# imdea-software/legosnark

Hardware: AMD Instinct MI355X
Metric: alt_bn128 G1 MSM point-scalar pairs/s at n=2^20 (higher is better)
Workload: dtype u32 limbs (254-bit Montgomery integers)

## Files before the change

legosnark_amd/csrc/msm.hip:

```cpp
#include <hip/hip_runtime.h>
#include <stdint.h>
#include <stdio.h>
#include <stdlib.h>
#include <string.h>
#include <algorithm>
#include <type_traits>
#include <vector>

#include "curves.h"
#include "fp29x2l.h"
#include "fs29.h"
#include "glv.h"
#include "msm.h"
#include "msm_plan.h"

namespace lsa {


template <class F, int K>
__global__ __launch_bounds__(256) void k_normalize(const Jac<F> *__restrict__ in, Aff<F> *__restrict__ out, size_t n) {
    size_t t = (size_t)blockIdx.x * blockDim.x + threadIdx.x;
    size_t base = t * K;
    if (base >= n) return;
    F prod[K];
// ... 198 lines not shown
__device__ __forceinline__ uint32_t block_exclusive_scan_256(uint32_t v, uint32_t *lds, uint32_t *total) {
    const unsigned lane = threadIdx.x & 63, wv = threadIdx.x >> 6;
    uint32_t incl = v;
#pragma unroll
    for (int d = 1; d < 64; d <<= 1) {
        uint32_t t = __shfl_up(incl, d, 64);
        if ((int)lane >= d) incl += t;
    }
    if (lane == 63) lds[wv] = incl;
    __syncthreads();
    uint32_t base = 0, tot = 0;
#pragma unroll
    for (unsigned w = 0; w < 4; w++) { uint32_t x = lds[w]; if (w < wv) base += x; tot += x; }
    __syncthreads();
    *total = tot;
    return base + incl - v;
}

__global__ __launch_bounds__(256) void k_scan_sums(const uint32_t *__restrict__ hist, uint32_t count, uint32_t *__restrict__ block_sums) {
    __shared__ uint32_t lds[4];
    const uint32_t base = blockIdx.x * SCAN_PER_BLOCK + threadIdx.x * 8;
    uint32_t s = 0;
#pragma unroll
    for (int j = 0; j < 8; j++) if (base + j < count) s += hist[base + j];
    uint32_t tot;
    (void)block_exclusive_scan_256(s, lds, &tot);
    if (threadIdx.x == 0) block_sums[blockIdx.x] = tot;
}

__global__ __launch_bounds__(256) void k_scan_blocks(uint32_t *__restrict__ block_sums, uint32_t nblocks) {
    __shared__ uint32_t lds[4];
    uint32_t v[4], s = 0;
#pragma unroll
    for (int j = 0; j < 4; j++) { uint32_t idx = threadIdx.x * 4 + j; v[j] = idx < nblocks ? block_sums[idx] : 0; s += v[j]; }
    uint32_t tot;
    uint32_t run = block_exclusive_scan_256(s, lds, &tot);
#pragma unroll
    for (int j = 0; j < 4; j++) { uint32_t idx = threadIdx.x * 4 + j; if (idx < nblocks) block_sums[idx] = run; run += v[j]; }
}

__global__ __launch_bounds__(256) void k_scan_final(const uint32_t *__restrict__ hist, const uint32_t *__restrict__ block_sums,
                                                    uint32_t count, uint32_t *__restrict__ offs) {
    __shared__ uint32_t lds[4];
    const uint32_t base = blockIdx.x * SCAN_PER_BLOCK + threadIdx.x * 8;
    uint32_t v[8], s = 0;
#pragma unroll
    for (int j = 0; j < 8; j++) { v[j] = (base + j < count) ? hist[base + j] : 0; s += v[j]; }
    uint32_t tot;
    uint32_t run = block_sums[blockIdx.x] + block_exclusive_scan_256(s, lds, &tot);
#pragma unroll
    for (int j = 0; j < 8; j++) { if (base + j < count) offs[base + j] = run; run += v[j]; }
}

__global__ __launch_bounds__(1024) void k_scatter(const int32_t *__restrict__ digits, const uint16_t *__restrict__ rank,
                                                  const uint32_t *__restrict__ offs, const uint32_t *__restrict__ tile_base,
                                                  size_t n, size_t npoints, uint32_t B, uint32_t ntiles, uint32_t *__restrict__ entries,
                                                  uint32_t win_stride) {
    extern __shared__ __attribute__((aligned(16))) uint32_t base[];
    const uint32_t t = blockIdx.x, k = blockIdx.y;
    const uint32_t *of = offs + (size_t)k * B;
    const uint32_t *tb = tile_base + ((size_t)k * ntiles + t) * B;
    for (uint32_t x = threadIdx.x; x < B; x += 1024) base[x] = of[x] + tb[x];
    __syncthreads();
    const size_t lo = (size_t)t * SORT_TILE;
    const size_t hi = lo + SORT_TILE < n ? lo + SORT_TILE : n;
    const int32_t *dg = digits + (size_t)k * n;
    const uint16_t *rk = rank + (size_t)k * n;
    for (size_t i = lo + threadIdx.x; i < hi; i += 1024) {
        int32_t sd = dg[i];
        if (sd != 0) {
            uint32_t b = (uint32_t)(sd < 0 ? -sd : sd) - 1;
            uint32_t pt = i < npoints ? (uint32_t)i : ((uint32_t)(i - npoints) | 0x40000000u);
            pt += k * win_stride;
            entries[base[b] + rk[i]] = pt | (sd < 0 ? 0x80000000u : 0u);
        }
    }
}

__global__ __launch_bounds__(1024) void k_tile_scan_rows(const uint16_t *__restrict__ tile_hist, uint32_t Bc, uint32_t R, uint32_t pitch,
                                                         uint32_t *__restrict__ tile_base, uint32_t *__restrict__ hist,
                                                         uint32_t *__restrict__ zero1, uint32_t *__restrict__ zeron, uint32_t nzero) {
    __builtin_amdgcn_s_setprio(3);
    if (blockIdx.x == 0) {
        if (threadIdx.x == 0) *zero1 = 0;
        for (uint32_t x = threadIdx.x; x < nzero; x += 1024) zeron[x] = 0;
    }
    __shared__ uint32_t part[32][33];
    const unsigned lane = threadIdx.x & 63, wv = threadIdx.x >> 6;
    const unsigned bl = lane & 31, grp = 2 * wv + (lane >> 5);
    const uint32_t b = blockIdx.x * 32 + bl;
    const uint32_t per = (R + 31) / 32, r0 = grp * per, r1 = r0 + per < R ? r0 + per : R;
    constexpr uint32_t MAXPER = 16;
    uint32_t v[MAXPER];
    uint32_t sum = 0;
    const bool in_regs = per <= MAXPER;
    if (in_regs) {
#pragma unroll
        for (uint32_t j = 0; j < MAXPER; j++) {
            const uint32_t r = r0 + j;
            v[j] = (b < Bc && r < r1) ? tile_hist[(size_t)r * pitch + b] : 0u;
        }
#pragma unroll
        for (uint32_t j = 0; j < MAXPER; j++) sum += v[j];
    } else if (b < Bc) {
        for (uint32_t r = r0; r < r1; r++) sum += tile_hist[(size_t)r * pitch + b];
    }
    part[grp][bl] = sum;
    __syncthreads();
    uint32_t run = 0, tot = 0;
#pragma unroll
    for (unsigned g2 = 0; g2 < 32; g2++) { uint32_t x = part[g2][bl]; if (g2 < grp) run += x; tot += x; }
    if (b < Bc) {
        if (in_regs) {
#pragma unroll
            for (uint32_t j = 0; j < MAXPER; j++) {
                const uint32_t r = r0 + j;
                if (r < r1) { tile_base[(size_t)r * pitch + b] = run; run += v[j]; }
            }
        } else {
            for (uint32_t r = r0; r < r1; r++) {
                const size_t idx = (size_t)r * pitch + b;
                tile_base[idx] = run;
                run += tile_hist[idx];
            }
        }
        if (grp == 0) hist[b] = tot;
    }
}

__device__ __forceinline__ uint32_t segment_of(const SegList &segs, uint32_t i) {
    uint32_t seg = 0;
    for (uint32_t j = 1; j < segs.nseg; j++) if (i >= segs.off[j]) seg = j;
    return seg;
}

__device__ __forceinline__ uint32_t xcd_tile(uint32_t bid, uint32_t ntiles) {
    const uint32_t q = ntiles >> 3, r = ntiles & 7u, x = bid & 7u, j = bid >> 3;
    return x * q + (x < r ? x : r) + j;
}

__global__ __launch_bounds__(1024) void k_hist_wide(const Fr *__restrict__ scalars, size_t n, SegList segs, WidePlan pl, uint32_t B,
                                                    uint32_t Bc, CoarseMap cm, uint32_t pitch, uint32_t tile,
                                                    uint16_t *__restrict__ tile_hist) {
    __builtin_amdgcn_s_setprio(3);
    extern __shared__ __attribute__((aligned(16))) uint32_t cnt2[];
    for (uint32_t x = threadIdx.x; x < (Bc + 1) / 2; x += blockDim.x) cnt2[x] = 0;
    __syncthreads();
    const uint32_t t = xcd_tile(blockIdx.x, gridDim.x);
    const size_t lo = (size_t)t * tile;
    for (uint32_t il = threadIdx.x; il < tile; il += blockDim.x) {
        const size_t i = lo + il;
        if (i >= n) break;
        const uint32_t seg = segment_of(segs, (uint32_t)i);
        wide_digits(scalars[i], pl, seg * B, [&](unsigned, int32_t sd) {
            if (sd != 0) {
                const uint32_t b = cm.bin((uint32_t)(sd < 0 ? -sd : sd) - 1);
                atomicAdd(&cnt2[b >> 1], 1u << ((b & 1) * 16));
            }
        });
    }
    __syncthreads();
    uint16_t *th = tile_hist + (size_t)t * pitch;
    const uint16_t *c16 = reinterpret_cast<const uint16_t *>(cnt2);
    for (uint32_t x = threadIdx.x; x < Bc; x += blockDim.x) th[x] = c16[x];
}

template <int REC>
// ... 32 lines not shown
    const size_t lo = (size_t)t * tile;
    for (uint32_t il = threadIdx.x; il < tile; il += 1024) {
        const size_t i = lo + il;
        if (i >= n) break;
        const uint32_t seg = segment_of(segs, (uint32_t)i);
        const uint32_t local = (uint32_t)i - segs.off[seg];
        wide_digits(scalars[i], pl, seg * B, [&](unsigned k, int32_t sd) {
            if (sd != 0) {
                const uint32_t b = (uint32_t)(sd < 0 ? -sd : sd) - 1;
                const uint32_t ent = (local + k * win_stride) | (sd < 0 ? 0x80000000u : 0u);
                if (REC == 1) ((uint64_t *)out)[atomicAdd(&base[b >> 7], 1u)] = ((uint64_t)(b & 127u) << 32) | ent;
                else if (REC == 2) ((uint32_t *)out)[atomicAdd(&base[b >> 6], 1u)] = (ent & 0x81ffffffu) | ((b & 63u) << 25);
                else ((uint32_t *)out)[atomicAdd(&base[b], 1u)] = ent;
            }
        });
    }
}

__device__ __forceinline__ uint32_t lds_inc_rank(uint32_t *counters, uint32_t idx) {
    const uint32_t first = (uint32_t)__builtin_amdgcn_readfirstlane((int)idx);
    const uint64_t active = __ballot(1), same = __ballot(idx == first);
    if (same == active) {
        const uint32_t rank = __builtin_amdgcn_mbcnt_hi((uint32_t)(active >> 32), __builtin_amdgcn_mbcnt_lo((uint32_t)active, 0u));
        uint32_t base = 0;
        if (rank == 0) base = atomicAdd(&counters[first], (uint32_t)__popcll(active));
        return (uint32_t)__builtin_amdgcn_readfirstlane((int)base) + rank;
    }
    return atomicAdd(&counters[idx], 1u);
}
__global__ __launch_bounds__(1024) void k_partition(const Fr *__restrict__ scalars, size_t n, SegList segs, WidePlan pl, uint32_t B, uint32_t Bc,
                                                    CoarseMap cm, uint32_t pitch, const uint16_t *__restrict__ tile_hist,
                                                    const uint32_t *__restrict__ hist_c, uint32_t *__restrict__ offs_c,
                                                    const uint32_t *__restrict__ tile_base, uint32_t *__restrict__ recs) {
    __builtin_amdgcn_s_setprio(3);
    extern __shared__ __attribute__((aligned(16))) uint32_t stage[];
    __shared__ uint32_t lstart[PART_SEGS + 1], lcur[PART_SEGS], gdst[PART_SEGS], wtot[2][PART_SEGS / 64];
    const uint32_t t = xcd_tile(blockIdx.x, gridDim.x);
    const unsigned lane = threadIdx.x & 63, wv = threadIdx.x >> 6;
    {
        uint32_t gv = 0, lv = 0;
        if (threadIdx.x < Bc) { gv = hist_c[threadIdx.x]; lv = tile_hist[(size_t)t * pitch + threadIdx.x]; }
        uint32_t gi = gv, li = lv;
#pragma unroll
        for (int d = 1; d < 64; d <<= 1) {
            const uint32_t a = __shfl_up(gi, d, 64), b = __shfl_up(li, d, 64);
            if ((int)lane >= d) { gi += a; li += b; }
        }
        if (wv < PART_SEGS / 64 && lane == 63) { wtot[0][wv] = gi; wtot[1][wv] = li; }
        __syncthreads();
        if (threadIdx.x < Bc) {
            uint32_t gex = gi - gv, lex = li - lv;
            for (unsigned w = 0; w < wv; w++) { gex += wtot[0][w]; lex += wtot[1][w]; }
            lstart[threadIdx.x] = lex;
            lcur[threadIdx.x] = lex;
            gdst[threadIdx.x] = gex + tile_base[(size_t)t * pitch + threadIdx.x];
            if (blockIdx.x == 0) offs_c[threadIdx.x] = gex;
            if (threadIdx.x == Bc - 1) lstart[Bc] = lex + lv;
        }
    }
    __syncthreads();
    const size_t lo = (size_t)t * PART_TILE;
    const uint32_t fine_bits = cm.sh_hi;
    const uint32_t tlow = t & ((1u << (16 - fine_bits)) - 1);
    for (uint32_t j = 0; j < PART_TILE / 1024; j++) {
        const uint32_t il = threadIdx.x + j * 1024;
        const size_t i = lo + il;
        if (i >= n) break;
        const uint32_t seg = segment_of(segs, (uint32_t)i);
        wide_digits(scalars[i], pl, seg * B, [&](unsigned k, int32_t sd) {
            if (sd != 0) {
                const uint32_t b = (uint32_t)(sd < 0 ? -sd : sd) - 1;
                const uint32_t pos = atomicAdd(&lcur[cm.bin(b)], 1u);
                stage[pos] = (tlow << (16 + fine_bits)) | (cm.fine(b) << 16) | (k << 12) | (sd < 0 ? 0x800u : 0u) | il;
            }
        });
    }
    __syncthreads();
    for (uint32_t sg = threadIdx.x >> 5; sg < Bc; sg += 32) {
        const uint32_t a = lstart[sg], e = lstart[sg + 1], g = gdst[sg];
        for (uint32_t x = a + (lane & 31); x < e; x += 32) recs[g + (x - a)] = stage[x];
    }
}

__global__ __launch_bounds__(1024) void k_fine_sort_part(const uint32_t *__restrict__ recs, const uint32_t *__restrict__ offs_c,
                                                         const uint32_t *__restrict__ hist_c, const uint32_t *__restrict__ tile_base,
                                                         uint32_t pitch, uint32_t T, CoarseMap cm, SegList segs, uint32_t win_stride, uint32_t stage_cap,
                                                         uint32_t *__restrict__ entries, uint32_t *__restrict__ hist, uint32_t *__restrict__ offs) {
    __builtin_amdgcn_s_setprio(3);
    extern __shared__ __attribute__((aligned(16))) uint32_t sm[];
    __shared__ uint32_t wsum[16];
    const uint32_t sg = blockIdx.x, lo = offs_c[sg], ns = hist_c[sg];
    const uint32_t fine_bits = cm.sh_hi, FM = 1u << fine_bits, fmask = FM - 1, tbits = 16 - fine_bits;
    const uint32_t F = 1u << cm.bits(sg), bucket0 = cm.first(sg);
    uint32_t *cnt = sm, *cur = sm + FM, *col = sm + 2 * FM, *stage = col + T + 1;
    const unsigned lane = threadIdx.x & 63, wv = threadIdx.x >> 6;
    for (uint32_t x = threadIdx.x; x < F; x += 1024) cnt[x] = 0;
    for (uint32_t x = threadIdx.x; x < T; x += 1024) col[x] = tile_base[(size_t)x * pitch + sg];
    if (threadIdx.x == 0) col[T] = ns;
    auto scan_counters = [&]() {
        const uint32_t per = (F + 1023) >> 10, f0 = threadIdx.x * per;
        uint32_t sum = 0;
        for (uint32_t q = 0; q < per; q++) if (f0 + q < F) sum += cnt[f0 + q];
        uint32_t incl = sum;
#pragma unroll
        for (int d = 1; d < 64; d <<= 1) {
            const uint32_t u = __shfl_up(incl, d, 64);
            if ((int)lane >= d) incl += u;
        }
        if (lane == 63) wsum[wv] = incl;
        __syncthreads();
        uint32_t run = incl - sum;
        for (unsigned w = 0; w < wv; w++) run += wsum[w];
        for (uint32_t q = 0; q < per; q++) {
            if (f0 + q >= F) break;
            const uint32_t c = cnt[f0 + q];
            cur[f0 + q] = run;
            hist[(size_t)bucket0 + f0 + q] = c;
            offs[(size_t)bucket0 + f0 + q] = lo + run;
            run += c;
        }
    };
    auto entry_of = [&](uint32_t r, uint32_t p2) {
        uint32_t a = 0, e = (T + (1u << tbits) - 1) >> tbits;
        while (e - a > 1) {
            const uint32_t m = (a + e) >> 1;
            if (col[m << tbits] <= p2) a = m; else e = m;
        }
        const uint32_t i = ((a << tbits) | (r >> (16 + fine_bits))) * PART_TILE + (r & 0x7ffu);
        const uint32_t local = i - segs.off[segment_of(segs, i)];
        return (local + ((r >> 12) & 15u) * win_stride) | ((r & 0x800u) << 20);
    };
    if (ns <= stage_cap) {
        constexpr uint32_t NR = PART_STAGE / 1024;
        uint32_t r[NR];
#pragma unroll
        for (uint32_t u = 0; u < NR; u++) { const uint32_t p2 = threadIdx.x + u * 1024; r[u] = p2 < ns ? recs[lo + p2] : 0u; }
        __syncthreads();
        uint16_t rk[NR];
#pragma unroll
        for (uint32_t u = 0; u < NR; u++) {
            rk[u] = 0;
            if (threadIdx.x + u * 1024 < ns) rk[u] = (uint16_t)atomicAdd(&cnt[(r[u] >> 16) & fmask], 1u);
        }
        __syncthreads();
        scan_counters();
        __syncthreads();
#pragma unroll
        for (uint32_t u = 0; u < NR; u++) {
            const uint32_t p2 = threadIdx.x + u * 1024;
            if (p2 < ns) stage[cur[(r[u] >> 16) & fmask] + rk[u]] = entry_of(r[u], p2);
        }
        __syncthreads();
        for (uint32_t x = threadIdx.x; x < ns; x += 1024) entries[lo + x] = stage[x];
        return;
    }
    __syncthreads();
    constexpr uint32_t UNR = 8;
    for (uint32_t p0 = threadIdx.x; p0 < ns; p0 += 1024 * UNR) {
        uint32_t r[UNR];
#pragma unroll
        for (uint32_t u = 0; u < UNR; u++) { const uint32_t p2 = p0 + u * 1024; r[u] = p2 < ns ? recs[lo + p2] : 0u; }
#pragma unroll
        for (uint32_t u = 0; u < UNR; u++) if (p0 + u * 1024 < ns) (void)lds_inc_rank(cnt, (r[u] >> 16) & fmask);
    }
    __syncthreads();
    scan_counters();
    __syncthreads();
    for (uint32_t p0 = threadIdx.x; p0 < ns; p0 += 1024 * UNR) {
        uint32_t r[UNR];
#pragma unroll
        for (uint32_t u = 0; u < UNR; u++) { const uint32_t p2 = p0 + u * 1024; r[u] = p2 < ns ? recs[lo + p2] : 0u; }
#pragma unroll
        for (uint32_t u = 0; u < UNR; u++) {
            const uint32_t p2 = p0 + u * 1024;
            if (p2 >= ns) break;
            entries[lo + lds_inc_rank(cur, (r[u] >> 16) & fmask)] = entry_of(r[u], p2);
        }
    }
}

template <class Rec>
struct RecOps;
template <>
struct RecOps<uint64_t> {
    static constexpr uint32_t NF = 128;
    static __device__ __forceinline__ uint32_t fine(uint64_t r) { return (uint32_t)(r >> 32); }
    static __device__ __forceinline__ uint32_t entry(uint64_t r) { return (uint32_t)r; }
};
template <>
struct RecOps<uint32_t> {
    static constexpr uint32_t NF = 64;
    static __device__ __forceinline__ uint32_t fine(uint32_t r) { return (r >> 25) & 63u; }
    static __device__ __forceinline__ uint32_t entry(uint32_t r) { return r & 0x81ffffffu; }
};
template <class Rec>
__global__ __launch_bounds__(1024) void k_fine_sort(const Rec *__restrict__ recs, const uint32_t *__restrict__ offs_c,
                                                    const uint32_t *__restrict__ hist_c, uint32_t *__restrict__ entries,
                                                    uint32_t *__restrict__ hist, uint32_t *__restrict__ offs) {
    using O = RecOps<Rec>;
    constexpr uint32_t NF = O::NF;
    __shared__ uint32_t cnt[NF], cur[NF];
    const uint32_t bin = blockIdx.x, lo = offs_c[bin], n = hist_c[bin];
    if (threadIdx.x < NF) cnt[threadIdx.x] = 0;
    __syncthreads();
    for (uint32_t j = threadIdx.x; j < n; j += 1024) atomicAdd(&cnt[O::fine(recs[lo + j])], 1u);
    __syncthreads();
    if (threadIdx.x < 64) {
        constexpr uint32_t PER = NF / 64;
        uint32_t c[PER], tot = 0;
#pragma unroll
        for (uint32_t q = 0; q < PER; q++) { c[q] = cnt[PER * threadIdx.x + q]; tot += c[q]; }
        uint32_t incl = tot;
#pragma unroll
        for (int d = 1; d < 64; d <<= 1) {
            uint32_t t = __shfl_up(incl, d, 64);
            if ((int)threadIdx.x >= d) incl += t;
        }
        uint32_t ex = incl - tot;
#pragma unroll
        for (uint32_t q = 0; q < PER; q++) {
            cur[PER * threadIdx.x + q] = ex;
            hist[(size_t)bin * NF + PER * threadIdx.x + q] = c[q];
            offs[(size_t)bin * NF + PER * threadIdx.x + q] = lo + ex;
            ex += c[q];
        }
    }
    __syncthreads();
    for (uint32_t j = threadIdx.x; j < n; j += 1024) {
        const Rec r = recs[lo + j];
        const uint32_t pos = atomicAdd(&cur[O::fine(r)], 1u);
        entries[lo + pos] = O::entry(r);
    }
}

__device__ __forceinline__ uint32_t size_bin(uint32_t cnt, uint32_t bin_shift) { return ((cnt - 1) >> bin_shift) + 1; }
template <class C>
__global__ __launch_bounds__(256) void k_size_hist(const uint32_t *__restrict__ hist, uint32_t nb, uint32_t thr, uint32_t *__restrict__ bin_count,
                                                   uint32_t group_size, uint32_t bin_shift) {
    bin_count += (group_size ? (blockIdx.x * 2048u) / group_size : 0u) * SIZE_BINS;
    __shared__ uint32_t lcnt[SIZE_BINS];
    for (uint32_t t = threadIdx.x; t < SIZE_BINS; t += 256) lcnt[t] = 0;
    __syncthreads();
    const uint32_t base = blockIdx.x * 2048 + threadIdx.x;
#pragma unroll
    for (int j = 0; j < 8; j++) {
        uint32_t g = base + j * 256;
        if (g < nb) { uint32_t cnt = hist[g]; if (cnt > 0 && cnt <= thr) atomicAdd(&lcnt[size_bin(cnt, bin_shift)], 1u); }
    }
    __syncthreads();
    for (uint32_t t = threadIdx.x; t < SIZE_BINS; t += 256) if (lcnt[t]) atomicAdd(&bin_count[t], lcnt[t]);
}
__global__ __launch_bounds__(256) void k_size_scan(const uint32_t *__restrict__ bin_count, uint32_t *__restrict__ bin_start, uint32_t ngroups) {
    __shared__ uint32_t lds[4];
    uint32_t carry = 0;
    for (uint32_t gidx = 0; gidx < ngroups; gidx++) {
        const uint32_t *bc = bin_count + gidx * SIZE_BINS;
        uint32_t *bs = bin_start + gidx * SIZE_BINS;
        uint32_t v[4], s = 0;
#pragma unroll
        for (int j = 0; j < 4; j++) {
            int bin = (int)SIZE_BINS - 1 - (int)(threadIdx.x * 4 + j);
            v[j] = (bin >= 1) ? bc[bin] : 0;
            s += v[j];
        }
        uint32_t tot;
        uint32_t run = carry + block_exclusive_scan_256(s, lds, &tot);
#pragma unroll
        for (int j = 0; j < 4; j++) {
            int bin = (int)SIZE_BINS - 1 - (int)(threadIdx.x * 4 + j);
            if (bin >= 1) bs[bin] = run;
            run += v[j];
        }
        carry += tot;
    }
    if (threadIdx.x == 0) bin_start[0] = carry;
}
template <class C>
__global__ __launch_bounds__(256) void k_size_scatter(const uint32_t *__restrict__ hist, uint32_t nb, uint32_t thr, const uint32_t *__restrict__ bin_start,
                                                      uint32_t *__restrict__ bin_cursor, uint32_t *__restrict__ perm,
                                                      uint32_t *__restrict__ heavy_list, uint32_t *__restrict__ heavy_count,
                                                      typename C::Acc *__restrict__ buckets, uint32_t group_size, uint32_t bin_shift,
                                                      uint32_t split) {
    const uint32_t goff = (group_size ? (blockIdx.x * 2048u) / group_size : 0u) * SIZE_BINS;
    bin_start += goff;
    bin_cursor += goff;
    __shared__ uint32_t lcnt[SIZE_BINS];
    for (uint32_t t = threadIdx.x; t < SIZE_BINS; t += 256) lcnt[t] = 0;
    __syncthreads();
    const uint32_t base = blockIdx.x * 2048 + threadIdx.x;
    uint32_t cnt[8], rank[8];
#pragma unroll
    for (int j = 0; j < 8; j++) {
        uint32_t g = base + j * 256;
        cnt[j] = 0; rank[j] = 0;
        if (g < nb) {
            cnt[j] = hist[g];
            if (cnt[j] == 0) { for (uint32_t h = 0; h < split; h++) buckets[(size_t)g * split + h] = C::inf(); }
            else if (cnt[j] > thr) heavy_list[atomicAdd(heavy_count, 1u)] = g;
            else rank[j] = atomicAdd(&lcnt[size_bin(cnt[j], bin_shift)], 1u);
        }
    }
    __syncthreads();
    for (uint32_t t = threadIdx.x; t < SIZE_BINS; t += 256) {
        uint32_t c = lcnt[t];
        lcnt[t] = c ? atomicAdd(&bin_cursor[t], c) : 0;
    }
    __syncthreads();
#pragma unroll
    for (int j = 0; j < 8; j++) {
        uint32_t g = base + j * 256;
        if (g < nb && cnt[j] > 0 && cnt[j] <= thr) {
            const uint32_t bin = size_bin(cnt[j], bin_shift);
            perm[bin_start[bin] + lcnt[bin] + rank[j]] = g;
        }
    }
}

template <class C, uint32_t ACC_SPLIT>
__device__ __forceinline__ void accumulate_body(const typename C::Base *__restrict__ bases, const uint32_t *__restrict__ entries,
                                                const uint32_t *__restrict__ offs, const uint32_t *__restrict__ hist,
                                                const uint32_t *__restrict__ perm, const uint32_t *__restrict__ nperm,
                                                typename C::Acc *__restrict__ buckets) {
    uint32_t t = blockIdx.x * blockDim.x + threadIdx.x;
    if (t >= *nperm * ACC_SPLIT) return;
    const uint32_t g = perm[t / ACC_SPLIT], part = t % ACC_SPLIT;
    const uint32_t cnt = hist[g];
    const uint32_t *e = entries + offs[g];
    constexpr bool ENDO = ACC_SPLIT != 1;
    typename C::Acc acc = C::inf();
    if (part < cnt) {
        uint32_t v = e[part];
        typename C::Base cur = bases[v & 0x3fffffffu];
        uint32_t j = part;
        if constexpr (C::HEAD) {
            if (j + ACC_SPLIT < cnt) {
                const uint32_t v1 = e[j + ACC_SPLIT];
                const typename C::Base b1 = bases[v1 & 0x3fffffffu];
                if (C::head_ok(cur, b1)) {
                    uint32_t vn = v1;
                    typename C::Base nxt = b1;
                    if (j + 2 * ACC_SPLIT < cnt) { vn = e[j + 2 * ACC_SPLIT]; nxt = bases[vn & 0x3fffffffu]; }
                    acc = C::template madd_head<ENDO>(cur, (v >> 31) != 0, ((v >> 30) & 1) != 0, b1, (v1 >> 31) != 0, ((v1 >> 30) & 1) != 0);
                    j += 2 * ACC_SPLIT;
                    v = vn;
                    cur = nxt;
                }
            }
        }
        for (; j < cnt; j += ACC_SPLIT) {
            uint32_t vn = v;
            typename C::Base nxt = cur;
            if (j + ACC_SPLIT < cnt) { vn = e[j + ACC_SPLIT]; nxt = bases[vn & 0x3fffffffu]; }
            acc = C::template madd<ENDO>(acc, cur, (v >> 31) != 0, ((v >> 30) & 1) != 0);
            v = vn;
            cur = nxt;
        }
    }
    buckets[(size_t)g * ACC_SPLIT + part] = acc;
}
template <class C, uint32_t ACC_SPLIT>
__global__ __launch_bounds__(256) void k_accumulate(const typename C::Base *__restrict__ bases, const uint32_t *__restrict__ entries,
                                                    const uint32_t *__restrict__ offs, const uint32_t *__restrict__ hist,
                                                    const uint32_t *__restrict__ perm, const uint32_t *__restrict__ nperm,
                                                    typename C::Acc *__restrict__ buckets) {
    accumulate_body<C, ACC_SPLIT>(bases, entries, offs, hist, perm, nperm, buckets);
}
__global__ __launch_bounds__(256) __attribute__((amdgpu_waves_per_eu(2, 2))) void k_accumulate_g2_occ2(
    const CurveG2::Base *__restrict__ bases, const uint32_t *__restrict__ entries, const uint32_t *__restrict__ offs,
    const uint32_t *__restrict__ hist, const uint32_t *__restrict__ perm, const uint32_t *__restrict__ nperm, CurveG2::Acc *__restrict__ buckets) {
    accumulate_body<CurveG2, 1u>(bases, entries, offs, hist, perm, nperm, buckets);
}

__global__ __launch_bounds__(256) void k_accumulate_g2_pair(const AffPackedG2 *__restrict__ bases, const uint32_t *__restrict__ entries,
                                                            const uint32_t *__restrict__ offs, const uint32_t *__restrict__ hist,
                                                            const uint32_t *__restrict__ perm, const uint32_t *__restrict__ nperm,
                                                            XYZZ29x2 *__restrict__ buckets) {
    const uint32_t t = blockIdx.x * blockDim.x + threadIdx.x, pr = t >> 1, part = t & 1;
    if (pr >= *nperm) return;
    const uint32_t g = perm[pr];
    const uint32_t cnt = hist[g];
    const uint32_t *e = entries + offs[g];
    struct Half { uint32_t x[8], y[8]; };
    auto fetch = [&](uint32_t v) {
        const AffPackedG2 &b = bases[v & 0x3fffffffu];
        Half h;
#pragma unroll
        for (int i = 0; i < 8; i++) { h.x[i] = b.w[part][i]; h.y[i] = b.w[2 + part][i]; }
        return h;
    };
    XyzzE<F29h> acc = XyzzE<F29h>::inf();
    uint32_t v = e[0];
    Half cur = fetch(v);
    for (uint32_t j = 0; j < cnt; j++) {
        uint32_t vn = v;
        Half nxt = cur;
        if (j + 1 < cnt) { vn = e[j + 1]; nxt = fetch(vn); }
        AffE<F29h> q = {{F29::unpack256(cur.x)}, {F29::unpack256(cur.y)}};
        if (!q.is_inf()) {
            if (v >> 31) q.y = sub_k<1>(F29h::zero(), q.y);
            acc = g2_madd(acc, q);
        }
        v = vn;
        cur = nxt;
    }
    F29 *o = reinterpret_cast<F29 *>(&buckets[g]);
    o[part] = acc.X.v;
    o[2 + part] = acc.Y.v;
    o[4 + part] = acc.ZZ.v;
    o[6 + part] = acc.ZZZ.v;
}

template <class A>
__device__ __forceinline__ A shfl_down_acc(const A &p, unsigned delta) {
    A r;
    constexpr int NW = sizeof(A) / 4;
    const uint32_t *src = reinterpret_cast<const uint32_t *>(&p);
    uint32_t *dst = reinterpret_cast<uint32_t *>(&r);
#pragma unroll
    for (int i = 0; i < NW; i++) dst[i] = __shfl_down(src[i], delta, 64);
    return r;
}

template <class C>
__device__ __forceinline__ typename C::Acc wave_sum(typename C::Acc v, unsigned lane) {
    for (unsigned d = 32; d >= 1; d >>= 1) {
        typename C::Acc t = shfl_down_acc(v, d);
        if (lane + d < 64) v = C::add(v, t);
    }
    return v;
}

__global__ __launch_bounds__(256) void k_heavy_plan(const uint32_t *__restrict__ hist, const uint32_t *__restrict__ heavy_list,
                                                    const uint32_t *__restrict__ heavy_count, uint32_t *__restrict__ chunk_off) {
    __shared__ uint32_t lds[4];
    __shared__ uint32_t s_chunk;
    const uint32_t nh = *heavy_count;
    uint32_t carry = 0;
    for (uint32_t base = 0; base < nh; base += 256) {
        uint32_t h = base + threadIdx.x;
        uint32_t tot;
        (void)block_exclusive_scan_256(h < nh ? hist[heavy_list[h]] : 0, lds, &tot);
        carry += tot;
    }
    if (threadIdx.x == 0) {
        uint32_t chunk = HEAVY_CHUNK;
        while (chunk < 4096u && carry / (2 * chunk) >= 2048u) chunk *= 2;
        s_chunk = chunk;
    }
    __syncthreads();
    const uint32_t chunk = s_chunk;
    carry = 0;
    for (uint32_t base = 0; base < nh; base += 256) {
        uint32_t h = base + threadIdx.x;
        uint32_t v = h < nh ? (hist[heavy_list[h]] + chunk - 1) / chunk : 0;
        uint32_t tot;
        uint32_t ex = block_exclusive_scan_256(v, lds, &tot);
        if (h < nh) chunk_off[h] = carry + ex;
        carry += tot;
    }
    if (threadIdx.x == 0) { chunk_off[nh] = carry; chunk_off[nh + 1] = chunk; }
}

template <class C>
__global__ __launch_bounds__(64) void k_accumulate_heavy(const typename C::Base *__restrict__ bases, const uint32_t *__restrict__ entries,
                                                         const uint32_t *__restrict__ offs, const uint32_t *__restrict__ hist,
                                                         const uint32_t *__restrict__ heavy_list, const uint32_t *__restrict__ heavy_count,
                                                         const uint32_t *__restrict__ chunk_off, typename C::Acc *__restrict__ partials) {
    const uint32_t nh = *heavy_count;
    if (nh == 0) return;
    const uint32_t total = chunk_off[nh], chunk = chunk_off[nh + 1];
    const unsigned lane = threadIdx.x;
    for (uint32_t v = blockIdx.x; v < total; v += gridDim.x) {
        uint32_t lo = 0, hi = nh;
        while (hi - lo > 1) { uint32_t mid = (lo + hi) >> 1; if (chunk_off[mid] <= v) lo = mid; else hi = mid; }
        const uint32_t g = heavy_list[lo];
        const uint32_t cnt = hist[g];
        const uint32_t start = (v - chunk_off[lo]) * chunk;
        const uint32_t end = start + chunk < cnt ? start + chunk : cnt;
        const uint32_t *e = entries + offs[g];
        typename C::Acc acc = C::inf();
        for (uint32_t j = start + lane; j < end; j += 64) {
            uint32_t w = e[j];
            acc = C::madd(acc, bases[w & 0x3fffffffu], (w >> 31) != 0, ((w >> 30) & 1) != 0);
        }
        acc = wave_sum<C>(acc, lane);
        if (lane == 0) partials[v] = acc;
    }
}

template <class C>
__global__ __launch_bounds__(64) void k_heavy_finish(const uint32_t *__restrict__ heavy_list, const uint32_t *__restrict__ heavy_count,
                                                     const uint32_t *__restrict__ chunk_off, const typename C::Acc *__restrict__ partials,
                                                     typename C::Acc *__restrict__ buckets, uint32_t split) {
    const uint32_t nh = *heavy_count;
    unsigned lane = threadIdx.x;
    for (uint32_t h = blockIdx.x; h < nh; h += gridDim.x) {
        typename C::Acc acc = C::inf();
        for (uint32_t v = chunk_off[h] + lane; v < chunk_off[h + 1]; v += 64) acc = C::add(acc, partials[v]);
        acc = wave_sum<C>(acc, lane);
        if (lane == 0) {
            buckets[(size_t)heavy_list[h] * split] = acc;
            for (uint32_t x = 1; x < split; x++) buckets[(size_t)heavy_list[h] * split + x] = C::inf();
        }
    }
}

template <class A>
__device__ __forceinline__ A select_acc(uint32_t mask, const A &a, const A &b) {
    A r;
    const uint32_t *pa = reinterpret_cast<const uint32_t *>(&a), *pb = reinterpret_cast<const uint32_t *>(&b);
    uint32_t *pr = reinterpret_cast<uint32_t *>(&r);
#pragma unroll
    for (int i = 0; i < (int)(sizeof(A) / 4); i++) pr[i] = (pa[i] & mask) | (pb[i] & ~mask);
    return r;
}
template <class A>
__device__ __forceinline__ void quadwave_weighted(A &acc, A &run, unsigned log_mult, unsigned lane) {
    const unsigned q = lane & 3, qi = lane >> 2;
    A s = A::inf();
#pragma unroll 1
    for (unsigned step = 0; step < 9; step++) {
        if (step == 4) {
            s = (qi == 0) ? A::inf() : run;
#pragma unroll 1
            for (unsigned i = 0; i < log_mult; i++) s = quad_dbl(s, q);
        }
        uint32_t m_run = step < 4 ? 0xffffffffu : 0u, m_s = step == 4 ? 0xffffffffu : 0u;
        asm volatile("" : "+v"(m_run), "+v"(m_s));
        const unsigned d = step < 4 ? (1u << step) : (step == 4 ? 0u : (8u >> (step - 5)));
        const A lhs = select_acc(m_run, run, acc);
        const A rhs = select_acc(m_s, s, shfl_down_acc(lhs, 4 * d));
        A r = lhs;
        if (qi + d < 16) r = quad_add(lhs, rhs, q);
        run = select_acc(m_run, r, run);
        acc = select_acc(m_run, acc, r);
    }
}

template <class C>
__global__ __launch_bounds__(64) void k_reduce1_lane(const typename C::Acc *__restrict__ buckets, uint32_t B, uint32_t L, uint32_t split,
                                                     typename C::Acc *__restrict__ out) {
    using A = typename C::Acc;
    const uint32_t t = blockIdx.x * 64 + threadIdx.x;
    if ((uint64_t)t * L >= B) return;
    A acc = A::inf(), run = A::inf();
// ... 552 lines not shown
    (void)hipFree(tmp);
    if (rc) return rc;
    if (e != hipSuccess) { set_error("precompute_windows: %s", hipGetErrorString(e)); return LSA_ERR_HIP; }
    return LSA_OK;
}
template <class F>
int precompute_window_step(void *d_table, size_t n, void *d_tmp, unsigned k, hipStream_t st) {
    using C = typename CurveOf<F>::type;
    const TableGrid grid = table_grid(n);
    if (n == 0 || k == 0 || k >= grid.ncopies) return LSA_OK;
    typename C::Base *tbl = (typename C::Base *)d_table;
    hipLaunchKernelGGL((k_shift_window<C>), dim3((unsigned)((n + 255) / 256)), dim3(256), 0, st, tbl + (size_t)(k - 1) * n, (Jac<F> *)d_tmp, n, grid.pos[k] - grid.pos[k - 1]);
    return prepare_bases<F>((const Jac<F> *)d_tmp, tbl + (size_t)k * n, n, st);
}
template int precompute_window_step<Fq>(void *, size_t, void *, unsigned, hipStream_t);
template int precompute_window_step<Fq2>(void *, size_t, void *, unsigned, hipStream_t);
template int precompute_windows<Fq>(void *, size_t, hipStream_t);
template int precompute_windows<Fq2>(void *, size_t, hipStream_t);

unsigned msm_field_mults_per_pair(size_t n, size_t table_n) {
    if (table_n && n >= switches().table_use_min) return wide_plan(table_n, n, 1, switches()).nwin * 10;
    return 16 * 10 + 8;
}

template <class A>
struct MsmBuffers {
    uint32_t *hist, *heavy_count, *offs, *bsum, *bin_count, *bin_start, *bin_cursor, *perm;
    int32_t *digits;
    uint16_t *rank, *tile_hist;
    uint32_t *tile_base, *entries, *heavy_list, *chunk_off;
    A *hpart;
    void *recs;
    uint32_t *hist_c, *offs_c;
    A *buckets, *wave_out, *window_sums;
    void *res;

    MsmBuffers(const PipelinePlan &p, void *front_ws, void *tail_ws) {
        char *ws = (char *)front_ws, *tws = (char *)tail_ws;
        hist = (uint32_t *)(ws + p.front[F_HIST]);
        heavy_count = hist + p.nb;
        offs = (uint32_t *)(ws + p.front[F_OFFS]);
        bsum = (uint32_t *)(ws + p.front[F_BSUM]);
        bin_count = (uint32_t *)(ws + p.front[F_BINS]);
        bin_start = bin_count + SIZE_BINS;
        bin_cursor = bin_start + SIZE_BINS;
        perm = (uint32_t *)(ws + p.front[F_PERM]);
        digits = (int32_t *)(ws + p.front[F_DIGITS]);
        rank = (uint16_t *)(ws + p.front[F_RANK]);
        tile_hist = (uint16_t *)(ws + p.front[F_THIST]);
        tile_base = (uint32_t *)(ws + p.front[F_TBASE]);
        entries = (uint32_t *)(ws + p.front[F_ENTRIES]);
        heavy_list = (uint32_t *)(ws + p.front[F_HEAVY]);
        chunk_off = (uint32_t *)(ws + p.front[F_CHOFF]);
        hpart = (A *)(ws + p.front[F_HPART]);
        recs = ws + p.front[F_RECS];
        hist_c = p.fine ? (uint32_t *)(ws + p.front[F_CHIST]) : hist;
        offs_c = p.fine ? (uint32_t *)(ws + p.front[F_COFFS]) : offs;
        buckets = (A *)(tws + p.tail[T_BUCKETS]);
        wave_out = (A *)(tws + p.tail[T_WAVE]);
        window_sums = (A *)(tws + p.tail[T_WIN]);
        res = tws + p.tail[T_RES];
    }
};

struct Marks {
    hipEvent_t *ev;
    void operator()(int i, hipStream_t s) const { if (ev) (void)hipEventRecord(ev[i], s); }
};

template <class C>
static void launch_sort(const PipelinePlan &p, const MsmBuffers<typename C::Acc> &b, const Fr *d_scalars, const SegList &segs, hipStream_t st,
                        const Marks &mark) {
    const size_t n = p.n;
    if (p.wide) {
        hipLaunchKernelGGL(k_hist_wide, dim3(p.wtiles), dim3(1024), p.lds_hist_wide, st, d_scalars, n, segs, p.pl, p.B, p.Bc, p.cm, p.pitch, p.wtile, b.tile_hist);
        mark(1, st);
        hipLaunchKernelGGL(k_tile_scan_rows, dim3((p.Bc + 31) / 32), dim3(1024), 0, st, b.tile_hist, p.Bc, p.wtiles, p.pitch, b.tile_base, b.hist_c, b.heavy_count,
                           b.bin_count, (uint32_t)(3 * SIZE_BINS));
        mark(2, st);
        if (p.part) {
            hipLaunchKernelGGL(k_partition, dim3(p.wtiles), dim3(1024), p.lds_partition, st, d_scalars, n, segs, p.pl, p.B, p.Bc, p.cm, p.pitch,
                               b.tile_hist, b.hist_c, b.offs_c, b.tile_base, (uint32_t *)b.recs);
            hipLaunchKernelGGL(k_fine_sort_part, dim3(p.Bc), dim3(1024), p.lds_fine_sort_part, st, (const uint32_t *)b.recs, b.offs_c, b.hist_c,
                               b.tile_base, p.pitch, p.wtiles, p.cm, segs, p.win_stride, p.stage_cap, b.entries, b.hist, b.offs);
        } else if (p.rec32) {
            hipLaunchKernelGGL(k_scatter_wide<2>, dim3(p.wtiles), dim3(1024), p.lds_scatter_wide, st, d_scalars, n, segs, p.pl, p.B, p.Bc, p.pitch, p.wtile, b.hist_c, b.offs_c, b.tile_base, b.recs, p.win_stride);
            hipLaunchKernelGGL(k_fine_sort<uint32_t>, dim3(p.Bc), dim3(1024), 0, st, (const uint32_t *)b.recs, b.offs_c, b.hist_c, b.entries, b.hist, b.offs);
        } else if (p.fine) {
            hipLaunchKernelGGL(k_scatter_wide<1>, dim3(p.wtiles), dim3(1024), p.lds_scatter_wide, st, d_scalars, n, segs, p.pl, p.B, p.Bc, p.pitch, p.wtile, b.hist_c, b.offs_c, b.tile_base, b.recs, p.win_stride);
            hipLaunchKernelGGL(k_fine_sort<uint64_t>, dim3(p.Bc), dim3(1024), 0, st, (const uint64_t *)b.recs, b.offs_c, b.hist_c, b.entries, b.hist, b.offs);
        } else {
            hipLaunchKernelGGL(k_scatter_wide<0>, dim3(p.wtiles), dim3(1024), p.lds_scatter_wide, st, d_scalars, n, segs, p.pl, p.B, p.Bc, p.pitch, p.wtile, b.hist_c, b.offs_c, b.tile_base, (void *)b.entries, p.win_stride);
        }
        mark(3, st);
    } else {
        hipLaunchKernelGGL((k_digits<C::GLV>), dim3((unsigned)((n + 255) / 256)), dim3(256), 0, st, d_scalars, n, p.c, p.nwin, b.digits);
        hipLaunchKernelGGL(k_rank, dim3(p.ntiles, p.nwin), dim3(1024), p.lds_rank, st, b.digits, p.nv, p.B, p.ntiles, b.rank, b.tile_hist, 0u);
        hipLaunchKernelGGL(k_tile_scan, dim3((p.nb + 255) / 256), dim3(256), 0, st, b.tile_hist, p.B, p.ntiles, p.nb, b.tile_base, b.hist);
        mark(1, st);
        hipLaunchKernelGGL(k_scan_sums, dim3(p.scan_blocks), dim3(256), 0, st, b.hist, p.nb, b.bsum);
        hipLaunchKernelGGL(k_scan_blocks, dim3(1), dim3(256), 0, st, b.bsum, p.scan_blocks);
        hipLaunchKernelGGL(k_scan_final, dim3(p.scan_blocks), dim3(256), 0, st, b.hist, b.bsum, p.nb, b.offs);
        mark(2, st);
        hipLaunchKernelGGL(k_scatter, dim3(p.ntiles, p.nwin), dim3(1024), p.lds_scatter, st, b.digits, b.rank, b.offs, b.tile_base, p.nv, n, p.B, p.ntiles, b.entries, 0u);
        mark(3, st);
    }
}

template <class C>
static int launch_accumulate(const PipelinePlan &p, const MsmBuffers<typename C::Acc> &b, const typename C::Base *d_bases, hipStream_t st, const Marks &mark) {
    constexpr bool g2 = std::is_same<C, CurveG2>::value;
    if (!p.wide || p.reuse_sort) {
        HIPCHK(hipMemsetAsync(b.heavy_count, 0, 4, st));
        HIPCHK(hipMemsetAsync(b.bin_count, 0, (size_t)3 * SIZE_BINS * 4, st));
    }
    const unsigned sb = (p.nb + 2047) / 2048;
    const uint32_t gsz = 0u, ngroups = 1;
    hipLaunchKernelGGL((k_size_hist<C>), dim3(sb), dim3(256), 0, st, b.hist, p.nb, p.heavy_threshold, b.bin_count, gsz, p.bin_shift);
    hipLaunchKernelGGL(k_size_scan, dim3(1), dim3(256), 0, st, b.bin_count, b.bin_start, ngroups);
    hipLaunchKernelGGL((k_size_scatter<C>), dim3(sb), dim3(256), 0, st, b.hist, p.nb, p.heavy_threshold, b.bin_start, b.bin_cursor, b.perm, b.heavy_list, b.heavy_count, b.buckets, gsz, p.bin_shift, p.split);
    mark(4, st);
    const dim3 one_lane((p.nb + 255) / 256), two_lanes((p.nb * 2 + 255) / 256);
    if (g2 && p.g2_pair) {
        if constexpr (g2) hipLaunchKernelGGL(k_accumulate_g2_pair, two_lanes, dim3(256), 0, st, d_bases, b.entries, b.offs, b.hist, b.perm, b.bin_start, b.buckets);
    } else if (g2 && p.split == 1) {
        if constexpr (g2) hipLaunchKernelGGL(k_accumulate_g2_occ2, one_lane, dim3(256), 0, st, d_bases, b.entries, b.offs, b.hist, b.perm, b.bin_start, b.buckets);
    } else if (p.split == 1) {
        hipLaunchKernelGGL((k_accumulate<C, 1u>), one_lane, dim3(256), 0, st, d_bases, b.entries, b.offs, b.hist, b.perm, b.bin_start, b.buckets);
    } else {
        hipLaunchKernelGGL((k_accumulate<C, 2u>), two_lanes, dim3(256), 0, st, d_bases, b.entries, b.offs, b.hist, b.perm, b.bin_start, b.buckets);
    }
    hipLaunchKernelGGL(k_heavy_plan, dim3(1), dim3(256), 0, st, b.hist, b.heavy_list, b.heavy_count, b.chunk_off);
    hipLaunchKernelGGL((k_accumulate_heavy<C>), dim3(4096), dim3(64), 0, st, d_bases, b.entries, b.offs, b.hist,
                       b.heavy_list, b.heavy_count, b.chunk_off, b.hpart);
    hipLaunchKernelGGL((k_heavy_finish<C>), dim3(256), dim3(64), 0, st, b.heavy_list, b.heavy_count, b.chunk_off, b.hpart, b.buckets, p.split);
    mark(5, st);
    return LSA_OK;
}

template <class C>
static int launch_tail(const PipelinePlan &p, const MsmBuffers<typename C::Acc> &b, Jac<typename C::Field> *d_out, hipStream_t tail, bool inline_tail,
                       bool lane_l1, TailBuf &tb, TailBuf &prev, const Marks &mark) {
    using A = typename C::Acc;
    using J = Jac<typename C::Field>;
    constexpr bool g1 = std::is_same<C, CurveG1>::value;
    if (p.big)
        hipLaunchKernelGGL((k_reduce1_lane<C>), dim3(p.kw * ((p.T + 63) / 64)), dim3(64), 0, tail, b.buckets, p.B, p.L, p.split, b.wave_out);
    else
        hipLaunchKernelGGL((k_reduce1<C>), dim3(p.kw * p.wpw), dim3(64), 0, tail, b.buckets, p.B, p.L, p.logL, p.wpw, p.split, b.wave_out);
    A *lvl_in = b.wave_out, *lvl_out = b.window_sums;
    uint32_t m = p.wpw, lm = p.big ? p.logL : p.logL + 4;
    J *res = inline_tail ? d_out : (J *)b.res;
    const auto level = [&](bool lane) {
        const uint32_t m_out = (m + 15) / 16;
        if (lane) hipLaunchKernelGGL((k_reduce2_lane<C>), dim3((m_out + 63) / 64), dim3(64), 0, tail, lvl_in, m, m_out, lm, lvl_out);
        else hipLaunchKernelGGL((k_reduce2<C>), dim3(p.kw * m_out), dim3(64), 0, tail, lvl_in, m, m_out, lm, lvl_out);
        std::swap(lvl_in, lvl_out);
        m = m_out;
        lm += 4;
    };
    level(lane_l1);
    if (p.bits_tail) {
        uint32_t nbits = 0;
        while ((1u << nbits) < m) nbits++;
        const uint32_t G = (m + 511) / 512;
        A *part = lvl_out;
        A *weighted = part + (size_t)(nbits + 1) * G;
        hipLaunchKernelGGL((k_reduce_bits_a<C>), dim3(nbits + 1, G), dim3(512), 0, tail, lvl_in, m, nbits, G, part);
        hipLaunchKernelGGL((k_reduce_bits_b<C>), dim3(nbits + 1), dim3(64), 0, tail, part, nbits, G, lm, weighted);
        mark(6, tail);
        hipLaunchKernelGGL((k_reduce_bits_c<C>), dim3(1), dim3(64), 0, tail, weighted, nbits + 1, res);
    } else {
        while (m > 1) level(false);
        mark(6, tail);
        if (p.wide && p.nseg > 1) {
            if constexpr (g1) hipLaunchKernelGGL(k_emit_g1, dim3(p.nseg), dim3(64), 0, tail, lvl_in, res);
            else hipLaunchKernelGGL(k_emit_g2, dim3(p.nseg), dim3(64), 0, tail, lvl_in, res);
        } else if constexpr (g1) {
            hipLaunchKernelGGL(k_fold_quad, dim3(1), dim3(64), 0, tail, lvl_in, p.kw, p.c, res);
        } else {
            hipLaunchKernelGGL(k_fold_quad_g2, dim3(1), dim3(64), 0, tail, lvl_in, p.kw, p.c, res);
        }
    }
    if (!inline_tail) {
        int rc = publish_order_large(tb, prev, tail);
        if (rc) return rc;
        hipLaunchKernelGGL(k_publish, dim3(1), dim3(256), 0, tail, (const uint32_t *)res, (uint32_t *)d_out, (unsigned)(p.nseg * sizeof(J) / 4));
    }
    mark(7, tail);
    return LSA_OK;
}

static int plan_error(const PipelinePlan &p) {
    switch (p.status) {
    case PLAN_OK: return LSA_OK;
    case PLAN_N_TOO_LARGE: set_error("msm: n too large (%zu)", p.n); break;
    case PLAN_SEGMENTS_NEED_COPIES: set_error("msm: segmented calls need bases with pre-shifted copies"); break;
    case PLAN_TABLE_TOO_LARGE: set_error("msm: base table too large for 30-bit entries"); break;
    case PLAN_BIN_SPACE: set_error("msm: %u segments of %u buckets exceed the bin space", p.nseg, p.B); break;
    }
    return LSA_ERR_INVALID;
}

template <class F>
static int msm_pipeline(const void *d_bases_v, size_t first, const Fr *d_scalars, const SegList &segs, Jac<F> *d_out, hipStream_t st,
                        size_t table_stride, bool reuse_sort = false, bool blocking = false) {
    using C = typename CurveOf<F>::type;
    using A = typename C::Acc;
    const typename C::Base *d_bases = (const typename C::Base *)d_bases_v + first;
    const MsmShape shape = {std::is_same<C, CurveG1>::value ? 1 : 2, sizeof(A), sizeof(Jac<F>), C::GLV, segs.off[segs.nseg], segs.nseg,
                            table_stride, blocking, reuse_sort};
    const PipelinePlan p = plan_pipeline(shape, switches());
    int rc = plan_error(p);
    if (rc) return rc;
    if (g_ws.ensure(p.front.total) != 0) { set_error("msm: workspace allocation of %zu bytes failed", p.front.total); return LSA_ERR_NOMEM; }
// ... 101 lines not shown
```

Baseline: 797.7 million.

## Fuse size-histogram, size-scan and heavy-plan into sort and scatter kernels

Bucket size-bin counts are now gathered inside the fine sort kernel when the partition path is used, so the separate size-histogram pass over all buckets is skipped. The size scan is folded into each size-scatter block, which now holds bin starts in shared memory and writes the bin_start[0] total (nperm). The heavy-plan kernel is folded into the last-arriving scatter block through an atomic block counter and acquire fence. This removes about three kernel launches and one pass over the histogram, at the cost of a redundant per-block scan and last-block synchronisation that relies on the second heavy_count word being cleared.

Result: no change. 795.6 million, median of 3 (-0.3%).

```diff
diff --git a/legosnark_amd/csrc/msm.hip b/legosnark_amd/csrc/msm.hip
--- a/legosnark_amd/csrc/msm.hip
+++ b/legosnark_amd/csrc/msm.hip
@@ -304,7 +304,7 @@
                                                          uint32_t *__restrict__ zero1, uint32_t *__restrict__ zeron, uint32_t nzero) {
     __builtin_amdgcn_s_setprio(3);
     if (blockIdx.x == 0) {
-        if (threadIdx.x == 0) *zero1 = 0;
+        if (threadIdx.x < 2) zero1[threadIdx.x] = 0;
         for (uint32_t x = threadIdx.x; x < nzero; x += 1024) zeron[x] = 0;
     }
     __shared__ uint32_t part[32][33];
@@ -503,13 +503,18 @@
     }
 }
 
+__device__ __forceinline__ uint32_t size_bin(uint32_t cnt, uint32_t bin_shift) { return ((cnt - 1) >> bin_shift) + 1; }
+
 __global__ __launch_bounds__(1024) void k_fine_sort_part(const uint32_t *__restrict__ recs, const uint32_t *__restrict__ offs_c,
                                                          const uint32_t *__restrict__ hist_c, const uint32_t *__restrict__ tile_base,
                                                          uint32_t pitch, uint32_t T, CoarseMap cm, SegList segs, uint32_t win_stride, uint32_t stage_cap,
-                                                         uint32_t *__restrict__ entries, uint32_t *__restrict__ hist, uint32_t *__restrict__ offs) {
+                                                         uint32_t *__restrict__ entries, uint32_t *__restrict__ hist, uint32_t *__restrict__ offs,
+                                                         uint32_t thr, uint32_t bin_shift, uint32_t *__restrict__ bin_count) {
     __builtin_amdgcn_s_setprio(3);
     extern __shared__ __attribute__((aligned(16))) uint32_t sm[];
     __shared__ uint32_t wsum[16];
+    __shared__ uint32_t lbin[SIZE_BINS];
+    for (uint32_t x = threadIdx.x; x < SIZE_BINS; x += 1024) lbin[x] = 0;
     const uint32_t sg = blockIdx.x, lo = offs_c[sg], ns = hist_c[sg];
     const uint32_t fine_bits = cm.sh_hi, FM = 1u << fine_bits, fmask = FM - 1, tbits = 16 - fine_bits;
     const uint32_t F = 1u << cm.bits(sg), bucket0 = cm.first(sg);
@@ -538,8 +543,12 @@
             cur[f0 + q] = run;
             hist[(size_t)bucket0 + f0 + q] = c;
             offs[(size_t)bucket0 + f0 + q] = lo + run;
+            if (c > 0 && c <= thr) atomicAdd(&lbin[size_bin(c, bin_shift)], 1u);
             run += c;
         }
+    };
+    auto flush_size_bins = [&]() {
+        for (uint32_t x = threadIdx.x; x < SIZE_BINS; x += 1024) if (lbin[x]) atomicAdd(&bin_count[x], lbin[x]);
     };
     auto entry_of = [&](uint32_t r, uint32_t p2) {
         uint32_t a = 0, e = (T + (1u << tbits) - 1) >> tbits;
@@ -566,6 +575,7 @@
         __syncthreads();
         scan_counters();
         __syncthreads();
+        flush_size_bins();
 #pragma unroll
         for (uint32_t u = 0; u < NR; u++) {
             const uint32_t p2 = threadIdx.x + u * 1024;
@@ -587,6 +597,7 @@
     __syncthreads();
     scan_counters();
     __syncthreads();
+    flush_size_bins();
     for (uint32_t p0 = threadIdx.x; p0 < ns; p0 += 1024 * UNR) {
         uint32_t r[UNR];
 #pragma unroll
@@ -654,11 +665,9 @@
     }
 }
 
-__device__ __forceinline__ uint32_t size_bin(uint32_t cnt, uint32_t bin_shift) { return ((cnt - 1) >> bin_shift) + 1; }
 template <class C>
 __global__ __launch_bounds__(256) void k_size_hist(const uint32_t *__restrict__ hist, uint32_t nb, uint32_t thr, uint32_t *__restrict__ bin_count,
-                                                   uint32_t group_size, uint32_t bin_shift) {
-    bin_count += (group_size ? (blockIdx.x * 2048u) / group_size : 0u) * SIZE_BINS;
+                                                   uint32_t bin_shift) {
     __shared__ uint32_t lcnt[SIZE_BINS];
     for (uint32_t t = threadIdx.x; t < SIZE_BINS; t += 256) lcnt[t] = 0;
     __syncthreads();
@@ -671,42 +680,63 @@
     __syncthreads();
     for (uint32_t t = threadIdx.x; t < SIZE_BINS; t += 256) if (lcnt[t]) atomicAdd(&bin_count[t], lcnt[t]);
 }
-__global__ __launch_bounds__(256) void k_size_scan(const uint32_t *__restrict__ bin_count, uint32_t *__restrict__ bin_start, uint32_t ngroups) {
+
+__device__ __forceinline__ void heavy_plan(const uint32_t *__restrict__ hist, const uint32_t *heavy_list, uint32_t nh, uint32_t *__restrict__ chunk_off,
+                                           uint32_t *lds, uint32_t *s_chunk) {
+    uint32_t carry = 0;
+    for (uint32_t base = 0; base < nh; base += 256) {
+        uint32_t h = base + threadIdx.x;
+        uint32_t tot;
+        (void)block_exclusive_scan_256(h < nh ? hist[heavy_list[h]] : 0, lds, &tot);
+        carry += tot;
+    }
+    if (threadIdx.x == 0) {
+        uint32_t chunk = HEAVY_CHUNK;
+        while (chunk < 4096u && carry / (2 * chunk) >= 2048u) chunk *= 2;
+        *s_chunk = chunk;
+    }
+    __syncthreads();
+    const uint32_t chunk = *s_chunk;
+    carry = 0;
+    for (uint32_t base = 0; base < nh; base += 256) {
+        uint32_t h = base + threadIdx.x;
+        uint32_t v = h < nh ? (hist[heavy_list[h]] + chunk - 1) / chunk : 0;
+        uint32_t tot;
+        uint32_t ex = block_exclusive_scan_256(v, lds, &tot);
+        if (h < nh) chunk_off[h] = carry + ex;
+        carry += tot;
+    }
+    if (threadIdx.x == 0) { chunk_off[nh] = carry; chunk_off[nh + 1] = chunk; }
+}
+
+template <class C>
+__global__ __launch_bounds__(256) void k_size_scatter(const uint32_t *__restrict__ hist, uint32_t nb, uint32_t thr, const uint32_t *__restrict__ bin_count,
+                                                      uint32_t *__restrict__ nperm, uint32_t *__restrict__ bin_cursor, uint32_t *__restrict__ perm,
+                                                      uint32_t *heavy_list, uint32_t *heavy_count,
+                                                      typename C::Acc *__restrict__ buckets, uint32_t bin_shift, uint32_t split,
+                                                      uint32_t *__restrict__ chunk_off) {
+    __shared__ uint32_t lcnt[SIZE_BINS], bstart[SIZE_BINS];
     __shared__ uint32_t lds[4];
-    uint32_t carry = 0;
-    for (uint32_t gidx = 0; gidx < ngroups; gidx++) {
-        const uint32_t *bc = bin_count + gidx * SIZE_BINS;
-        uint32_t *bs = bin_start + gidx * SIZE_BINS;
+    __shared__ uint32_t s_flag[2];
+    for (uint32_t t = threadIdx.x; t < SIZE_BINS; t += 256) lcnt[t] = 0;
+    {
         uint32_t v[4], s = 0;
 #pragma unroll
         for (int j = 0; j < 4; j++) {
             int bin = (int)SIZE_BINS - 1 - (int)(threadIdx.x * 4 + j);
-            v[j] = (bin >= 1) ? bc[bin] : 0;
+            v[j] = (bin >= 1) ? bin_count[bin] : 0;
             s += v[j];
         }
         uint32_t tot;
-        uint32_t run = carry + block_exclusive_scan_256(s, lds, &tot);
+        uint32_t run = block_exclusive_scan_256(s, lds, &tot);
 #pragma unroll
         for (int j = 0; j < 4; j++) {
             int bin = (int)SIZE_BINS - 1 - (int)(threadIdx.x * 4 + j);
-            if (bin >= 1) bs[bin] = run;
+            if (bin >= 1) bstart[bin] = run;
             run += v[j];
         }
-        carry += tot;
-    }
-    if (threadIdx.x == 0) bin_start[0] = carry;
-}
-template <class C>
-__global__ __launch_bounds__(256) void k_size_scatter(const uint32_t *__restrict__ hist, uint32_t nb, uint32_t thr, const uint32_t *__restrict__ bin_start,
-                                                      uint32_t *__restrict__ bin_cursor, uint32_t *__restrict__ perm,
-                                                      uint32_t *__restrict__ heavy_list, uint32_t *__restrict__ heavy_count,
-                                                      typename C::Acc *__restrict__ buckets, uint32_t group_size, uint32_t bin_shift,
-                                                      uint32_t split) {
-    const uint32_t goff = (group_size ? (blockIdx.x * 2048u) / group_size : 0u) * SIZE_BINS;
-    bin_start += goff;
-    bin_cursor += goff;
-    __shared__ uint32_t lcnt[SIZE_BINS];
-    for (uint32_t t = threadIdx.x; t < SIZE_BINS; t += 256) lcnt[t] = 0;
+        if (blockIdx.x == 0 && threadIdx.x == 0) *nperm = tot;
+    }
     __syncthreads();
     const uint32_t base = blockIdx.x * 2048 + threadIdx.x;
     uint32_t cnt[8], rank[8];
@@ -717,7 +747,7 @@
         if (g < nb) {
             cnt[j] = hist[g];
             if (cnt[j] == 0) { for (uint32_t h = 0; h < split; h++) buckets[(size_t)g * split + h] = C::inf(); }
-            else if (cnt[j] > thr) heavy_list[atomicAdd(heavy_count, 1u)] = g;
+            else if (cnt[j] > thr) __hip_atomic_store(&heavy_list[atomicAdd(heavy_count, 1u)], g, __ATOMIC_RELAXED, __HIP_MEMORY_SCOPE_AGENT);
             else rank[j] = atomicAdd(&lcnt[size_bin(cnt[j], bin_shift)], 1u);
         }
     }
@@ -732,9 +762,23 @@
         uint32_t g = base + j * 256;
         if (g < nb && cnt[j] > 0 && cnt[j] <= thr) {
             const uint32_t bin = size_bin(cnt[j], bin_shift);
-            perm[bin_start[bin] + lcnt[bin] + rank[j]] = g;
-        }
-    }
+            perm[bstart[bin] + lcnt[bin] + rank[j]] = g;
+        }
+    }
+    asm volatile("s_waitcnt vmcnt(0)" ::: "memory");
+    __syncthreads();
+    if (threadIdx.x == 0) {
+        const bool last = __hip_atomic_fetch_add(heavy_count + 1, 1u, __ATOMIC_RELAXED, __HIP_MEMORY_SCOPE_AGENT) == gridDim.x - 1;
+        s_flag[0] = last ? __hip_atomic_load(heavy_count, __ATOMIC_RELAXED, __HIP_MEMORY_SCOPE_AGENT) + 1 : 0u;
+    }
+    __syncthreads();
+    if (s_flag[0] == 0) return;
+    const uint32_t nh = s_flag[0] - 1;
+    if (nh) {
+        if (threadIdx.x == 0) { __builtin_amdgcn_fence(__ATOMIC_ACQUIRE, "agent"); asm volatile("s_waitcnt vmcnt(0)" ::: "memory"); }
+        __syncthreads();
+    }
+    heavy_plan(hist, heavy_list, nh, chunk_off, lds, &s_flag[1]);
 }
 
 template <class C, uint32_t ACC_SPLIT>
@@ -851,37 +895,6 @@
     return v;
 }
 
-__global__ __launch_bounds__(256) void k_heavy_plan(const uint32_t *__restrict__ hist, const uint32_t *__restrict__ heavy_list,
-                                                    const uint32_t *__restrict__ heavy_count, uint32_t *__restrict__ chunk_off) {
-    __shared__ uint32_t lds[4];
-    __shared__ uint32_t s_chunk;
-    const uint32_t nh = *heavy_count;
-    uint32_t carry = 0;
-    for (uint32_t base = 0; base < nh; base += 256) {
-        uint32_t h = base + threadIdx.x;
-        uint32_t tot;
-        (void)block_exclusive_scan_256(h < nh ? hist[heavy_list[h]] : 0, lds, &tot);
-        carry += tot;
-    }
-    if (threadIdx.x == 0) {
-        uint32_t chunk = HEAVY_CHUNK;
-        while (chunk < 4096u && carry / (2 * chunk) >= 2048u) chunk *= 2;
-        s_chunk = chunk;
-    }
-    __syncthreads();
-    const uint32_t chunk = s_chunk;
-    carry = 0;
-    for (uint32_t base = 0; base < nh; base += 256) {
-        uint32_t h = base + threadIdx.x;
-        uint32_t v = h < nh ? (hist[heavy_list[h]] + chunk - 1) / chunk : 0;
-        uint32_t tot;
-        uint32_t ex = block_exclusive_scan_256(v, lds, &tot);
-        if (h < nh) chunk_off[h] = carry + ex;
-        carry += tot;
-    }
-    if (threadIdx.x == 0) { chunk_off[nh] = carry; chunk_off[nh + 1] = chunk; }
-}
-
 template <class C>
 __global__ __launch_bounds__(64) void k_accumulate_heavy(const typename C::Base *__restrict__ bases, const uint32_t *__restrict__ entries,
                                                          const uint32_t *__restrict__ offs, const uint32_t *__restrict__ hist,
@@ -1600,7 +1613,8 @@
             hipLaunchKernelGGL(k_partition, dim3(p.wtiles), dim3(1024), p.lds_partition, st, d_scalars, n, segs, p.pl, p.B, p.Bc, p.cm, p.pitch,
                                b.tile_hist, b.hist_c, b.offs_c, b.tile_base, (uint32_t *)b.recs);
             hipLaunchKernelGGL(k_fine_sort_part, dim3(p.Bc), dim3(1024), p.lds_fine_sort_part, st, (const uint32_t *)b.recs, b.offs_c, b.hist_c,
-                               b.tile_base, p.pitch, p.wtiles, p.cm, segs, p.win_stride, p.stage_cap, b.entries, b.hist, b.offs);
+                               b.tile_base, p.pitch, p.wtiles, p.cm, segs, p.win_stride, p.stage_cap, b.entries, b.hist, b.offs,
+                               p.heavy_threshold, p.bin_shift, b.bin_count);
         } else if (p.rec32) {
             hipLaunchKernelGGL(k_scatter_wide<2>, dim3(p.wtiles), dim3(1024), p.lds_scatter_wide, st, d_scalars, n, segs, p.pl, p.B, p.Bc, p.pitch, p.wtile, b.hist_c, b.offs_c, b.tile_base, b.recs, p.win_stride);
             hipLaunchKernelGGL(k_fine_sort<uint32_t>, dim3(p.Bc), dim3(1024), 0, st, (const uint32_t *)b.recs, b.offs_c, b.hist_c, b.entries, b.hist, b.offs);
@@ -1629,14 +1643,14 @@
 static int launch_accumulate(const PipelinePlan &p, const MsmBuffers<typename C::Acc> &b, const typename C::Base *d_bases, hipStream_t st, const Marks &mark) {
     constexpr bool g2 = std::is_same<C, CurveG2>::value;
     if (!p.wide || p.reuse_sort) {
-        HIPCHK(hipMemsetAsync(b.heavy_count, 0, 4, st));
+        HIPCHK(hipMemsetAsync(b.heavy_count, 0, 8, st));
         HIPCHK(hipMemsetAsync(b.bin_count, 0, (size_t)3 * SIZE_BINS * 4, st));
     }
     const unsigned sb = (p.nb + 2047) / 2048;
-    const uint32_t gsz = 0u, ngroups = 1;
-    hipLaunchKernelGGL((k_size_hist<C>), dim3(sb), dim3(256), 0, st, b.hist, p.nb, p.heavy_threshold, b.bin_count, gsz, p.bin_shift);
-    hipLaunchKernelGGL(k_size_scan, dim3(1), dim3(256), 0, st, b.bin_count, b.bin_start, ngroups);
-    hipLaunchKernelGGL((k_size_scatter<C>), dim3(sb), dim3(256), 0, st, b.hist, p.nb, p.heavy_threshold, b.bin_start, b.bin_cursor, b.perm, b.heavy_list, b.heavy_count, b.buckets, gsz, p.bin_shift, p.split);
+    if (!p.part || p.reuse_sort)
+        hipLaunchKernelGGL((k_size_hist<C>), dim3(sb), dim3(256), 0, st, b.hist, p.nb, p.heavy_threshold, b.bin_count, p.bin_shift);
+    hipLaunchKernelGGL((k_size_scatter<C>), dim3(sb), dim3(256), 0, st, b.hist, p.nb, p.heavy_threshold, b.bin_count, b.bin_start, b.bin_cursor, b.perm,
+                       b.heavy_list, b.heavy_count, b.buckets, p.bin_shift, p.split, b.chunk_off);
     mark(4, st);
     const dim3 one_lane((p.nb + 255) / 256), two_lanes((p.nb * 2 + 255) / 256);
     if (g2 && p.g2_pair) {
@@ -1648,7 +1662,6 @@
     } else {
         hipLaunchKernelGGL((k_accumulate<C, 2u>), two_lanes, dim3(256), 0, st, d_bases, b.entries, b.offs, b.hist, b.perm, b.bin_start, b.buckets);
     }
-    hipLaunchKernelGGL(k_heavy_plan, dim3(1), dim3(256), 0, st, b.hist, b.heavy_list, b.heavy_count, b.chunk_off);
     hipLaunchKernelGGL((k_accumulate_heavy<C>), dim3(4096), dim3(64), 0, st, d_bases, b.entries, b.offs, b.hist,
                        b.heavy_list, b.heavy_count, b.chunk_off, b.hpart);
     hipLaunchKernelGGL((k_heavy_finish<C>), dim3(256), dim3(64), 0, st, b.heavy_list, b.heavy_count, b.chunk_off, b.hpart, b.buckets, p.split);
```
